# knights-lab/BURST

Hardware: AMD Instinct MI355X
Metric: aligned reads/sec (node), 100-bp synthetic reads @0.98 id vs RefSeq stand-in .edx/.acx (DB15), -m BEST; 1 GPU (higher is better)
Workload: dtype u32 bit-vectors (u8 edit distances)

## Files before the change

burst_amd/csrc/bhip_align.hip:

```cpp
#include "bhip_handle.h"
#include "bhip_pf_select.h"

__global__ void k_hit_count(const BhipHit *__restrict__ hits, uint32_t n, const uint32_t *__restrict__ n_dev, uint32_t *__restrict__ cnt, uint32_t *__restrict__ rank) {
	if (n_dev) n = *n_dev < n ? *n_dev : n;
	for (uint32_t i = blockIdx.x * blockDim.x + threadIdx.x; i < n; i += gridDim.x * blockDim.x) rank[i] = atomicAdd(&cnt[hits[i].q], 1u);
}
__global__ void k_hit_scatter(const BhipHit *__restrict__ in, uint32_t n, const uint32_t *__restrict__ n_dev, const uint32_t *__restrict__ off, const uint32_t *__restrict__ rank,
                              BhipHit *__restrict__ out, const uint32_t *__restrict__ qmap) {
	if (n_dev) n = *n_dev < n ? *n_dev : n;
	for (uint32_t i = blockIdx.x * blockDim.x + threadIdx.x; i < n; i += gridDim.x * blockDim.x) {
		BhipHit h = in[i];
		const uint32_t dst = off[h.q] + rank[i];
		if (qmap) h.q = qmap[h.q];
		out[dst] = h;
	}
}
__global__ void k_junk_adjust_raw(BhipRawHit *__restrict__ raw, const uint32_t *__restrict__ n_raw_dev, uint32_t raw_cap, const uint8_t *__restrict__ nx) {
	uint32_t n = *n_raw_dev;
	if (n > raw_cap) n = raw_cap;
	for (uint32_t i = blockIdx.x * blockDim.x + threadIdx.x; i < n; i += gridDim.x * blockDim.x) { const uint32_t x = nx[raw[i].q]; raw[i].ed += x; raw[i].m += x; }
}
__global__ void k_junk_adjust_best(uint32_t *__restrict__ best, const uint8_t *__restrict__ nx_six, uint32_t s0, uint32_t s1) {
	for (uint32_t s = s0 + blockIdx.x * blockDim.x + threadIdx.x; s < s1; s += gridDim.x * blockDim.x)
		if (nx_six[s] && best[s] != 0xFFFFFFFFu) best[s] += nx_six[s];
// ... 152 lines not shown
	memset(&fa, 0, sizeof fa);
	if (hipFuncGetAttributes(&fa, fn) != hipSuccess) return 4;
	return bhip_resident_blocks(threads, {fa.numRegs, fa.sharedSizeBytes}, dyn_lds);
}
template <auto FN> static BhipKernelRes kernel_res() {
	static const BhipKernelRes res = [] { hipFuncAttributes fa; memset(&fa, 0, sizeof fa);
		return hipFuncGetAttributes(&fa, (const void *)FN) == hipSuccess ? BhipKernelRes{fa.numRegs, fa.sharedSizeBytes} : BhipKernelRes{0, 0}; }();
	return res;
}

static void launch_window(Handle *h, Lane *L, hipStream_t wst, int cls, int NWP, uint32_t grid_cap, const BhipWin *wins, const uint32_t *n_wins, Counters *dc) {
	const uint32_t *six = six_or_null(h);
	const uint4 *ref = ref_args(h).chunks();
	const int NWc = kClasses[cls];
	const int min_class = h->opt_no_band ? 0 : NWc >= 8 ? 3 : NWc >= 6 ? 2 : NWc >= 4 ? 1 : 0;
	for_each_int(BwList{}, [&](auto bw) {
		constexpr int BW = decltype(bw)::value;
		if (min_class < BW - 1) return;
		uint32_t per_cu = blocks_per_cu((const void *)k_myers_window_band<BW>, 64u, 0);
		if (h->opt_band_blocks > 0) per_cu = (uint32_t)h->opt_band_blocks;
		const uint32_t grid = (uint32_t)h->n_cu * per_cu * (uint32_t)h->opt_oversub;
		hipLaunchKernelGGL(k_myers_window_band<BW>, dim3(grid), dim3(64), 0, wst, wins, n_wins, (uint32_t)L->win_cap, NWP, NWc, L->peq.as<uint32_t>(), six,
			ref, L->raw.as<BhipRawHit>(), &dc->n_raw, (uint32_t)L->raw_cap, h->best.as<uint32_t>(), &dc->wcol_sum, dc->win_class_seen);
	});
	dispatch_int(NwList{}, NWc, [&](auto nw) {
		constexpr int N = decltype(nw)::value;
		const uint32_t thr = N <= 8 ? 64u : 256u;
		const uint32_t grid = std::min<uint32_t>(grid_cap * (256u / thr), (uint32_t)h->n_cu * blocks_per_cu((const void *)k_myers_window<N>, thr, 0));
		hipLaunchKernelGGL(k_myers_window<N>, dim3(grid), dim3(thr), 0, wst, wins, n_wins, (uint32_t)L->win_cap, NWP, min_class, L->peq.as<uint32_t>(), six,
			ref, L->raw.as<BhipRawHit>(), &dc->n_raw, (uint32_t)L->raw_cap, h->best.as<uint32_t>(), &dc->wcol_sum, dc->win_class_seen);
	});
}


static int upload_queries(Handle *h, const uint8_t *q_codes, const uint64_t *q_off, const uint16_t *q_emac,
                          const uint32_t *q_six, const uint8_t *q_rc, uint32_t n_q) {
	const uint64_t nb = q_off[n_q];
	int rc;
	h->cur->st_has_junk = false;
	h->cur->st_maxlen = 0; h->cur->st_maxE = 0;
	for (uint32_t i = 0; i < n_q; ++i) {
		h->cur->st_maxlen = std::max<uint32_t>(h->cur->st_maxlen, (uint32_t)(q_off[i + 1] - q_off[i]));
		h->cur->st_maxE = std::max<uint32_t>(h->cur->st_maxE, q_emac[i]);
	}
	if ((rc = h->cur->qcodes.reserve(nb + 16))) return rc;
// ... 622 lines not shown
	for (uint32_t l = 0; l < b.nl; ++l) {
		Lane *L = h->lanes[l];
		const bool cq_min_only = !b.all_hits && h->opt_pf_cw == 2 && L->pf_algo_used == 3;
		if (L->n_entries && L->pf_algo == 0 && !cq_min_only && L->hc.ent_read > 100000 && (double)L->hc.surv_sum > (b.all_hits ? 0.20 : 0.50) * (double)L->hc.ent_read) L->pf_algo = 1;
	}
}
static void print_chain_counters(const Handle *h, const BatchCall &b) {
	for (uint32_t l = 0; l < b.nl; ++l) {
		const Lane *L = h->lanes[l];
		if (!L->n_entries) continue;
		fprintf(stderr, "[bhip] lane %u: %llu list records, %llu survived the counting filter, next prefilter algorithm %d\n", l, (unsigned long long)L->hc.ent_read, (unsigned long long)L->hc.surv_sum, L->pf_algo);
		for (int cls = 0; cls < kNumClasses; ++cls) if (L->npf[cls] + L->nex[cls])
			fprintf(stderr, "[bhip] lane %u class NW=%d: prefiltered %u exhaustive %u maxE %u maxwords %u | tasks %u + deferred %u (kept %u) clump pairs %u windows %u + %u | fallback queries(last class) %u raw %u\n",
				l, kClasses[cls], L->npf[cls], L->nex[cls], L->maxE[cls], L->maxwords[cls], L->hc.n_tasks_cls[cls], L->hc.n_tasks2_cls[cls], L->hc.n_tasks2k_cls[cls], L->hc.n_cand_cls[cls], L->hc.n_wins_cls[cls], L->hc.n_wins2_cls[cls], L->hc.n_fb, L->hc.n_raw);
		if (L->hc.n_fb) fprintf(stderr, "[bhip] lane %u: %u queries overflowed the first prefilter pass, %u the second (dense fallback)\n", l, L->hc.n_fb, L->hc.n_fb2);
		const uint32_t *rs = L->hc.n_rs;
		fprintf(stderr, "[bhip] lane %u: re-scorer bands 4:%u 6:%u 8:%u 12:%u 16:%u 24:%u 32:%u 40:%u 48:%u lds:%u scratch:%u\n",
			l, rs[0], rs[1], rs[2], rs[3], rs[4], rs[5], rs[6], rs[7], rs[8], rs[9], L->hc.n_wide);
		if (h->opt_rescore_reg) {
			static const char *const qf_name[BHIP_QF_COUNT] = {"dword", "lds", "chunk"};
			const BhipQueryFetch *f = L->qfetch;
			fprintf(stderr, "[bhip] lane %u: re-scorer query fetch 4-8:%s/%u 12:%s/%u 16-24:%s/%u 32-48:%s/%u\n", l, qf_name[f[0].form], f[0].lds_bytes,
				qf_name[f[3].form], f[3].lds_bytes, qf_name[f[1].form], f[1].lds_bytes, qf_name[f[2].form], f[2].lds_bytes);
		}
	}
}
static int grow_lane_capacities(Handle *h, const BatchCall &b) {
	bool redo = false;
	for (uint32_t l = 0; l < b.nl; ++l) {
		Lane *L = h->lanes[l];
// ... 337 lines not shown
```

burst_amd/csrc/bhip_handle.h:

```cpp
#ifndef BHIP_HANDLE_H
#define BHIP_HANDLE_H
#include <hip/hip_runtime.h>
#include <hipcub/hipcub.hpp>
#include <string>
#include <stdint.h>
#include <stdio.h>
#include <stdarg.h>
#include <stdlib.h>
#include <string.h>
#include <algorithm>
#include <vector>
#include <mutex>
#include <atomic>
#include <chrono>
#include <thread>
#include "burst_hip.h"
#include "bhip_internal.h"
#include "bhip_fetch_plan.h"

__global__ void k_acx_offsets(const uint32_t *, uint64_t, int, uint32_t *, unsigned long long *);
__global__ void k_acx_lines(const uint32_t *, uint64_t, int, unsigned long long *, uint4 *);
__global__ void k_acx_decode(const uint8_t *, const unsigned long long *, const uint32_t *, BhipAcxView, uint64_t, int, uint32_t, uint32_t *, uint32_t *);
__global__ void k_transpose_refs(const uint8_t *, const uint64_t *, const uint32_t *, const uint64_t *, uint32_t, uint4 *);
__global__ void k_build_peq(const uint8_t *, const uint64_t *, const uint32_t *, uint32_t, int, int, BhipMatchMask, uint32_t *, const uint32_t *, uint32_t, uint32_t);
// ... 3 lines not shown
__global__ void k_prefilter_hash(const uint8_t *, const uint64_t *, const uint16_t *, const uint32_t *, uint32_t, BhipAcxView, int,
	const uint32_t *, uint32_t, uint2 *, uint32_t *, uint32_t *, uint32_t, unsigned long long *, const uint32_t *, uint32_t *, uint32_t *);
template <typename CNT> __global__ void k_prefilter_wave(const uint8_t *, const uint64_t *, const uint16_t *, const uint32_t *, uint32_t,
	BhipAcxView, int, uint32_t, const uint32_t *, uint32_t, uint2 *, uint32_t *, uint32_t *, uint32_t, unsigned long long *, const uint32_t *,
	const uint32_t *, const uint32_t *);
template <int NW> __global__ void k_myers(const uint2 *, const uint32_t *, uint64_t, uint32_t, uint32_t, const uint32_t *, const uint32_t *,
	const uint64_t *, const uint16_t *, const uint32_t *, const uint4 *, const uint64_t *, const uint32_t *, uint32_t,
	BhipRawHit *, uint32_t *, uint32_t, uint32_t *, uint8_t *, unsigned long long *, unsigned long long *);
__global__ void k_myers_long(const uint2 *, const uint32_t *, uint64_t, uint32_t, uint32_t, const uint32_t *, const uint32_t *,
	const uint64_t *, const uint16_t *, const uint32_t *, const uint4 *, const uint64_t *, const uint32_t *, uint32_t,
	BhipRawHit *, uint32_t *, uint32_t, uint32_t *, uint8_t *, unsigned long long *, unsigned long long *, uint32_t);
template <int NWP> __global__ void k_myers_prefix(const uint2 *, const uint32_t *, uint64_t, uint32_t, uint32_t, const uint32_t *, const uint32_t *,
	const uint64_t *, const uint16_t *, const uint4 *, const uint64_t *, const uint32_t *, uint32_t, BhipWin *, uint32_t *, uint32_t,
	unsigned long long *, unsigned long long *, uint32_t *, const uint32_t *);
template <int NW> __global__ void k_myers_window(const BhipWin *, const uint32_t *, uint32_t, int, int, const uint32_t *, const uint32_t *,
	const uint4 *, BhipRawHit *, uint32_t *, uint32_t, uint32_t *, unsigned long long *, const uint32_t *);
template <int BW> __global__ void k_myers_window_band(const BhipWin *, const uint32_t *, uint32_t, int, int, const uint32_t *, const uint32_t *,
	const uint4 *, BhipRawHit *, uint32_t *, uint32_t, uint32_t *, unsigned long long *, const uint32_t *);
__global__ void k_extract_kmers(const uint4 *, const uint64_t *, const uint32_t *, const uint64_t *, uint32_t, uint32_t, int, unsigned long long *, uint16_t *, uint32_t *);
__global__ void k_attach_masks(BhipAcxView, uint64_t, const unsigned long long *, const uint16_t *, uint32_t, const uint32_t *, uint32_t *, uint32_t, uint32_t);
template <int HTB> __global__ void k_prefilter_mask(const uint2 *, const uint2 *, uint32_t, uint32_t, const uint32_t *, const uint32_t *, uint32_t, const uint32_t *, uint32_t,
	uint2 *, uint32_t *, uint32_t, unsigned long long *, uint32_t *, uint32_t *, unsigned long long *, unsigned long long *, unsigned long long *,
	uint2 *, uint32_t *, uint32_t);
template <int MODE, int BIG> __global__ void k_prefilter_cq(const uint2 *, const uint2 *, uint32_t, uint32_t, const uint32_t *, const uint32_t *, uint32_t, const uint32_t *, uint32_t,
	uint2 *, uint32_t *, uint32_t, unsigned long long *, uint32_t *, uint32_t *, unsigned long long *, unsigned long long *, unsigned long long *, unsigned long long *,
	uint2 *, uint32_t *, int, const uint32_t *, const uint32_t *, int);
template <int MODE, int BIG> __global__ void k_prefilter_cw(const uint2 *, const uint2 *, uint32_t, uint32_t, const uint32_t *, const uint32_t *, uint32_t, const uint32_t *, uint32_t,
	uint2 *, uint32_t *, uint32_t, unsigned long long *, uint32_t *, uint32_t *, unsigned long long *, unsigned long long *, unsigned long long *, unsigned long long *,
	uint2 *, uint32_t *, int, const uint32_t *, const uint32_t *, int);
__global__ void k_task_filter(const uint2 *, const uint32_t *, uint32_t, const uint32_t *, const uint32_t *, const uint32_t *, uint2 *, uint32_t *);
__global__ void k_seed_ranges(const uint8_t *, const uint64_t *, const uint32_t *, uint32_t, BhipAcxView, int, const uint32_t *, uint32_t, uint2 *, uint2 *, const uint32_t *, uint32_t, const uint16_t *, uint4 *, const uint32_t *, uint32_t, uint32_t, BhipAlt);
template <int NWP> __global__ void k_myers_prefix_task(const uint2 *, const uint32_t *, uint32_t, const uint32_t *, const uint32_t *, const uint64_t *,
	const uint16_t *, const uint4 *, const uint64_t *, const uint32_t *, BhipWin *, uint32_t *, uint32_t, unsigned long long *, uint32_t *, const uint4 *, const uint32_t *);
// ... 151 lines not shown

struct Counters {
	uint32_t n_cand, n_raw, n_out, n_wide, err, pad0;
	uint32_t n_cand_cls[8];
	uint32_t n_wins_cls[8];
	uint32_t n_fb, n_fb2;
	uint32_t n_tasks_cls[8];
	uint32_t n_tasks2_cls[8];
	uint32_t n_tasks2k_cls[8];
	uint32_t n_wins2_cls[8];
	uint32_t n_rs[12];
	unsigned long long wcol_sum, tcol_sum, unit_sum;
	unsigned long long col_sum, qlen_sum, ent_read, scratch_used;
	unsigned long long surv_sum;
	uint32_t win_class_seen[4];
};

struct StageSlot {
	DBuf qcodes, qcodes4, qlen16, qoff, qemac, qsix, qrc, qflags, qmap, off_raw, plan, qpack, key, key_sorted, idx, idx_sorted, sort_tmp, info;
	DBuf qcodes_s, qoff_s, qemac_s, qpack_s, nx, nx_six;
	BhipStageInfo *info_pinned = nullptr;
	hipEvent_t ev_begin = nullptr, ev_done = nullptr, ev_copied = nullptr;
	int state = 0;
	uint64_t seq = 0;
	bool resolved = false;
	bool st_valid = false, st_has_six = false, st_has_rc = false, st_has_junk = false, has_flags = false, has_qmap = false;
	uint32_t st_nq = 0, st_nshared = 0, st_maxlen = 0, st_maxE = 0, st_lanes = 1;
	float st_ms_h2d = 0, st_ms_copy = 0, st_ms_route = 0;
	std::vector<BhipQuerySpan> spans;
	const uint32_t *six_explicit = nullptr;
// ... 94 lines not shown
	const uint16_t *s_emac() const { return cur->st_has_junk ? cur->qemac_s.as<uint16_t>() : cur->qemac.as<uint16_t>(); }
	const uint32_t *s_pack() const { return cur->st_has_junk ? cur->qpack_s.as<uint32_t>() : cur->qpack.as<uint32_t>(); }
	DBuf sort_keys, sort_keys2, sort_idx, sort_tmp, out_sorted, out_sorted2, sort_scratch;
	uint64_t out_cap = 1 << 20;
	std::vector<uint32_t> h_clump_len;
	BhipStats stats;
	std::vector<Lane *> lanes;
	int opt_two_stage = 1;
	int opt_prefilter_stride = 0;
	int opt_lanes = 1;
	int opt_sweep_blocks = 8;
	uint32_t peq_rows = 16;
	int opt_oversub = 2;
	int opt_band_blocks = 0;
	int opt_no_band = 0;
	int opt_async_d2h = 0, out_idx = 0;
	hipStream_t copy_stream = nullptr;
	hipEvent_t ev_sorted = nullptr, ev_copied[2] = {nullptr, nullptr};
	bool copy_pending[2] = {false, false};
	void *reg_ptr[2] = {nullptr, nullptr}; size_t reg_bytes[2] = {0, 0};
	int last_out = 0;
	uint64_t last_n_out = 0;
	int opt_prune = 1;
	int opt_lane_min = 32768;
	int opt_rescore_reg = 1;
	int opt_fetch_once = 1;
	int opt_pf_waves = 0;
	int opt_pf_algo = -1;
	int opt_pf_table = 0;
	int opt_pf_cw = 2;
// ... 39 lines not shown
```

burst_amd/csrc/bhip_init.hip:

```cpp
#include "bhip_handle.h"

static thread_local char g_err[512] = "";

__global__ void k_ref_symbol_scan(const uint32_t *__restrict__ w, uint64_t n_words, uint32_t *__restrict__ flag) {
	uint32_t any = 0;
	for (uint64_t i = blockIdx.x * (uint64_t)blockDim.x + threadIdx.x; i < n_words; i += (uint64_t)gridDim.x * blockDim.x) {
		const uint32_t d = w[i];
		any |= (d | ((d << 1) & ((d << 2) | (d << 3)))) & 0x88888888u;
	}
	if (any) *flag = 1u;
}
int bhip_fail_msg(int code, const char *fmt, ...) {
	va_list ap; va_start(ap, fmt); vsnprintf(g_err, sizeof g_err, fmt, ap); va_end(ap);
	return code;
}

extern "C" const char *bhip_last_error(void) { return g_err; }
extern "C" int bhip_abi_version(void) { return BHIP_ABI_VERSION; }
std::atomic<int> &bhip_vmm_peer_access_flag() { return bhip_vmm_peer_access(); }

static void lane_destroy(Lane *L) {
	if (!L) return;
	DBuf *all[] = {&L->peq, &L->peqp, &L->cand, &L->candcnt, &L->wins, &L->raw, &L->wide, &L->scratch, &L->fb_list, &L->gcnt, &L->counters, &L->tasks, &L->tasks2, &L->tasks2k, &L->wins2, &L->rs_lists};
	for (DBuf *b : all) b->release();
// ... 185 lines not shown
		h->opt_prefilter_stride = (int)value; return BHIP_OK;
	}
	if (!strcmp(name, "two_stage")) { h->opt_two_stage = value != 0; return BHIP_OK; }
	if (!strcmp(name, "host_routing")) { h->opt_host_routing = value != 0; return BHIP_OK; }
	if (!strcmp(name, "discard_staged")) { for (StageSlot &S : h->slots) if (S.state == 1) S.state = 0; h->res_valid = false; return BHIP_OK; }
	if (!strcmp(name, "lane_masks")) { h->opt_lane_masks = value != 0; return BHIP_OK; }
	if (!strcmp(name, "sweep_blocks")) { if (value < 1 || value > 8) return fail(BHIP_E_ARG, "sweep_blocks must be 1 .. 8"); h->opt_sweep_blocks = (int)value; return BHIP_OK; }
	if (!strcmp(name, "lane_min_entries")) { if (value < 1) return fail(BHIP_E_ARG, "lane_min_entries must be >= 1"); h->opt_lane_min = (int)value; return BHIP_OK; }
	if (!strcmp(name, "async_d2h")) { h->opt_async_d2h = value != 0; return BHIP_OK; }
	if (!strcmp(name, "seed_ahead")) { h->opt_seed_ahead = value != 0; return BHIP_OK; }
	if (!strcmp(name, "peq_ahead_blocks")) { if (value < 1 || value > 16) return fail(BHIP_E_ARG, "peq_ahead_blocks must be 1 .. 16"); h->opt_peq_ahead_blocks = (int)value; return BHIP_OK; }
	if (!strcmp(name, "seed_ahead_blocks")) { if (value < 0 || value > 64) return fail(BHIP_E_ARG, "seed_ahead_blocks must be 0 .. 64"); h->opt_seed_ahead_blocks = (int)value; return BHIP_OK; }
	if (!strcmp(name, "band_blocks")) { if (value < 0 || value > 1024) return fail(BHIP_E_ARG, "band_blocks must be 0 .. 1024"); h->opt_band_blocks = (int)value; return BHIP_OK; }
	if (!strcmp(name, "oversub")) { if (value < 1 || value > 16) return fail(BHIP_E_ARG, "oversub must be 1 .. 16"); h->opt_oversub = (int)value; return BHIP_OK; }
	if (!strcmp(name, "band")) { h->opt_no_band = value == 0; return BHIP_OK; }
	if (!strcmp(name, "prune")) { h->opt_prune = value != 0; return BHIP_OK; }
	if (!strcmp(name, "rescore_reg")) { h->opt_rescore_reg = value != 0; return BHIP_OK; }
	if (!strcmp(name, "fetch_once")) { h->opt_fetch_once = value != 0; return BHIP_OK; }
	if (!strcmp(name, "seed_min_need")) { if (value < -1 || value > 255) return fail(BHIP_E_ARG, "seed_min_need must be -1 (by rule) or 0 .. 255"); h->opt_seed_min_need = (int)value; return BHIP_OK; }
	if (!strcmp(name, "seed_drop_len")) { if (value < 0 || value > (1 << 24)) return fail(BHIP_E_ARG, "seed_drop_len must be 0 .. 2^24"); h->opt_seed_drop_len = (int)value; return BHIP_OK; }
	if (!strcmp(name, "prefilter_waves")) { if (value < 0 || value > 16) return fail(BHIP_E_ARG, "prefilter_waves must be 0 .. 16"); h->opt_pf_waves = (int)value; return BHIP_OK; }
	if (!strcmp(name, "prefilter_algo")) { if (value < -1 || value > 1) return fail(BHIP_E_ARG, "prefilter_algo must be -1, 0 or 1"); h->opt_pf_algo = (int)value; return BHIP_OK; }
	if (!strcmp(name, "prefilter_table")) { if (value != 0 && (value < 9 || value > 11)) return fail(BHIP_E_ARG, "prefilter_table must be 0, 9, 10 or 11"); h->opt_pf_table = (int)value; return BHIP_OK; }
	if (!strcmp(name, "prefilter_cw")) { if (value < 0 || value > 2) return fail(BHIP_E_ARG, "prefilter_cw must be 0, 1 or 2"); h->opt_pf_cw = (int)value; return BHIP_OK; }
	if (!strcmp(name, "prefilter_bytes")) { h->opt_pf_bytes = value != 0; return BHIP_OK; }
	if (!strcmp(name, "prefilter_rb")) { if (value != 0 && (value < 2 || value > 4)) return fail(BHIP_E_ARG, "prefilter_rb must be 0, 2, 3 or 4"); h->opt_pf_rb = (int)value; return BHIP_OK; }
	if (!strcmp(name, "cov_event_cap")) { if (value < 0) return fail(BHIP_E_ARG, "cov_event_cap must be >= 0 bytes (0 = a fifth of the free memory)"); h->opt_cov_event_cap = value; return BHIP_OK; }
	if (!strcmp(name, "em_weak_hash")) { h->opt_em_weak_hash = value != 0; return BHIP_OK; }
	if (!strcmp(name, "em_thread_max")) { if (value < 0 || value > 64) return fail(BHIP_E_ARG, "em_thread_max must be 0 (built in) .. 64"); h->opt_em_thread_max = (int)value; return BHIP_OK; }
	if (!strcmp(name, "em_wave_max")) { if (value < 0 || value > (1 << 24)) return fail(BHIP_E_ARG, "em_wave_max must be 0 (built in) .. 2^24"); h->opt_em_wave_max = (int)value; return BHIP_OK; }
// ... 19 lines not shown
```

burst_amd/csrc/bhip_internal.h:

```cpp
#ifndef BHIP_INTERNAL_H
#define BHIP_INTERNAL_H
#include <stdint.h>

struct BhipMatchMask { uint16_t m[16]; };

struct BhipRawHit {
	uint32_t q;
	uint32_t refIx;
	uint32_t ed;
	uint32_t e_first;
	uint32_t e_last;
	uint32_t m;
	uint32_t L;
	uint32_t six;
	uint64_t rbase;
};

#define BHIP_WIN_GMASK 0x3FFFFFFFu
struct BhipWin {
	uint32_t li;
	uint32_t refIx;
	uint32_t g_first, g_last;
	uint32_t q;
	uint32_t mE;
	uint32_t nchunks;
	uint32_t L;
	uint64_t rbase;
	uint32_t six;
	uint32_t pad2;
};
__host__ __device__ inline uint32_t bhip_win_class(uint32_t g_first, uint32_t g_last, uint32_t E) {
	const uint64_t diags = 8ull * (g_last - g_first) + 8u + 2u * E;
	return diags <= 26 ? 0u : diags <= 58 ? 1u : diags <= 90 ? 2u : 3u;
}

#define BHIP_PLAN_STRIDE(p) ((p) & 255u)
#define BHIP_PLAN_NEED(p)   (((p) >> 8) & 0xFFFFu)
#define BHIP_PLAN_X(p)      (((p) >> 24) & 15u)
#define BHIP_PLAN_USED(p)   ((p) >> 28)
#define BHIP_EXPAND_SLOTS 8u
struct BhipAlt { uint8_t n[16]; uint8_t base[16]; };

template <class Sym>
__host__ __device__ inline uint32_t bhip_word_class(Sym sym, uint32_t p, uint32_t K, const BhipAlt &A, uint32_t &amb_k, uint32_t &extra) {
	uint32_t namb = 0, bad = 0;
	amb_k = 0; extra = 0;
	for (uint32_t k = 0; k < K; ++k) {
		const uint32_t n = A.n[sym(p + k) & 15u];
		if (n == 0u) bad = 1u;
// ... 82 lines not shown
```

burst_amd/csrc/bhip_kernels.hip:

```cpp
#include <hip/hip_runtime.h>
#include <stdint.h>
#include <type_traits>
#include "burst_hip.h"
#include "bhip_internal.h"
#include "bhip_fetch_plan.h"

__global__ void k_transpose_refs(const uint8_t *__restrict__ src, const uint64_t *__restrict__ src_off,
                                 const uint32_t *__restrict__ clump_len, const uint64_t *__restrict__ dst_off,
                                 uint32_t n_clumps, uint4 *__restrict__ dst_lane) {
	const uint32_t z = threadIdx.x & 15, g = threadIdx.x >> 4, gpb = blockDim.x >> 4;
	for (uint32_t c = blockIdx.x; c < n_clumps; c += gridDim.x) {
		const uint32_t L = clump_len[c], nrows = (L + 1) >> 1, nchunks = (L + 31) >> 5;
		const uint8_t *s = src + src_off[c] * 16;
		for (uint32_t t = g; t < nchunks; t += gpb) {
			uint32_t w[4] = {0, 0, 0, 0};
			#pragma unroll
			for (int i = 0; i < 16; ++i) {
				uint32_t row = 16 * t + i;
				uint32_t b = row < nrows ? s[(uint64_t)row * 16 + z] : 0u;
				w[i >> 2] |= b << (8 * (i & 3));
			}
			dst_lane[dst_off[c] * 16 + (uint64_t)z * nchunks + t] = make_uint4(w[0], w[1], w[2], w[3]);
		}
	}
// ... 457 lines not shown
		for (int t = 0; t < 8; ++t) if (keep[t]) out[s_base + rank[t]] = tk[t];
		__syncthreads();
	}
}

#define BHIP_INST_PREFIX_TASK(NWP) \
	template __global__ void k_myers_prefix_task<NWP>(const uint2 *, const uint32_t *, uint32_t, const uint32_t *, const uint32_t *, const uint64_t *, \
		const uint16_t *, const uint4 *, const uint64_t *, const uint32_t *, BhipWin *, uint32_t *, uint32_t, unsigned long long *, uint32_t *, const uint4 *, const uint32_t *);
BHIP_INST_PREFIX_TASK(1) BHIP_INST_PREFIX_TASK(2) BHIP_INST_PREFIX_TASK(3) BHIP_INST_PREFIX_TASK(4) BHIP_INST_PREFIX_TASK(6)

template <int NW>
__global__ __launch_bounds__(256) void k_myers_window(
		const BhipWin *__restrict__ wins, const uint32_t *__restrict__ n_wins_dev, uint32_t win_cap, int NWP, int min_class,
		const uint32_t *__restrict__ peq, const uint32_t *__restrict__ qsix, const uint4 *__restrict__ ref,
		BhipRawHit *__restrict__ raw, uint32_t *__restrict__ n_raw, uint32_t raw_cap, uint32_t *__restrict__ best,
		unsigned long long *__restrict__ wcol_sum, const uint32_t *__restrict__ cls_seen) {
	if (min_class > 0) {
		uint32_t any = 0;
		for (int c = min_class; c < 4; ++c) any |= cls_seen[c];
		if (!any) return;
	}
	constexpr bool LDS_TAB = NW <= 8;
	__shared__ uint32_t s_tab[LDS_TAB ? 4 * NW : 1][LDS_TAB ? 64 : 1];
	uint32_t n = *n_wins_dev;
	if (n > win_cap) n = win_cap;
	unsigned long long my_cols = 0;
	for (uint32_t i = blockIdx.x * blockDim.x + threadIdx.x; i < n; i += gridDim.x * blockDim.x) {
		const BhipWin w = wins[i];
		if ((int)(w.g_first >> 30) < min_class) continue;
		const uint32_t li = w.li, q = w.q;
		const uint32_t m = w.mE & 0xFFFFu, E = w.mE >> 16;
		const uint32_t P = m < 32u * (uint32_t)NWP ? m : 32u * (uint32_t)NWP;
		const uint32_t nchunks = w.nchunks, gA8 = w.g_first & BHIP_WIN_GMASK;
		const int col_lo = (int)(gA8 * 8 + 2) - (int)(P + E), col_hi = (int)((w.g_last + 1) * 8 + (m - P) + E);
		const uint32_t c_lo = col_lo > 1 ? (uint32_t)(col_lo - 1) : 0u;
		uint32_t c_hi = (uint32_t)(col_hi - 1);
		if (c_hi >= nchunks * 32) c_hi = nchunks * 32 - 1;
		const uint32_t tA = c_lo >> 5, tB = c_hi >> 5, gA = (c_lo & 31u) >> 3, gE = (c_hi & 31u) >> 3;
		uint32_t Pv[NW], Mv[NW];
		#pragma unroll
		for (int k = 0; k < NW; ++k) {
			const int lo = 32 * NW - (int)m - 32 * k;
			Pv[k] = lo <= 0 ? 0xFFFFFFFFu : (lo >= 32 ? 0u : (0xFFFFFFFFu << lo));
			Mv[k] = 0;
// ... 33 lines not shown
				}
			}
		}
		my_cols += ((tB * 4 + gE) - (tA * 4 + gA) + 1) * 8;
		if ((uint32_t)bestS <= E) {
			const uint32_t pos = atomicAdd(n_raw, 1u);
			if (pos < raw_cap) {
				BhipRawHit h; h.q = q; h.refIx = w.refIx; h.ed = (uint32_t)bestS; h.e_first = first; h.e_last = last;
				h.m = m; h.L = w.L; h.six = w.six; h.rbase = w.rbase;
				raw[pos] = h;
			}
			if (best) atomicMin(&best[w.six], (uint32_t)bestS);
		}
	}
	if (wcol_sum && my_cols) atomicAdd(wcol_sum, my_cols);
}

template <int BW>
__global__ __launch_bounds__(64) void k_myers_window_band(
		const BhipWin *__restrict__ wins, const uint32_t *__restrict__ n_wins_dev, uint32_t win_cap, int NWP, int NW,
		const uint32_t *__restrict__ peq, const uint32_t *__restrict__ qsix, const uint4 *__restrict__ ref,
		BhipRawHit *__restrict__ raw, uint32_t *__restrict__ n_raw, uint32_t raw_cap, uint32_t *__restrict__ best,
		unsigned long long *__restrict__ wcol_sum, const uint32_t *__restrict__ cls_seen) {
	if (BW > 2 && !cls_seen[BW - 2]) return;
	__shared__ uint32_t s_tab[4 * BW][64];
	const uint32_t tid = threadIdx.x;
	uint32_t n = *n_wins_dev;
	if (n > win_cap) n = win_cap;
	unsigned long long my_cols = 0;
#ifndef WB_PREFETCH
#define WB_PREFETCH 0
#endif
#if WB_PREFETCH
	BhipWin w_next;
	if (blockIdx.x * 64u + tid < n) w_next = wins[blockIdx.x * 64u + tid];
#endif
	for (uint32_t i = blockIdx.x * 64u + tid; i < n; i += gridDim.x * 64u) {
#if WB_PREFETCH
		const BhipWin w = w_next;
		if (i + gridDim.x * 64u < n) w_next = wins[i + gridDim.x * 64u];
#else
		const BhipWin w = wins[i];
#endif
		if (w.g_first >> 30 != (uint32_t)(BW - 2)) continue;
		const uint32_t m = w.mE & 0xFFFFu, E = w.mE >> 16, g_first = w.g_first & BHIP_WIN_GMASK;
		const uint32_t P = m < 32u * (uint32_t)NWP ? m : 32u * (uint32_t)NWP;
		const uint32_t nchunks = w.nchunks;
		const int col_lo = (int)(g_first * 8 + 2) - (int)(P + E), col_hi = (int)((w.g_last + 1) * 8 + (m - P) + E);
		const uint32_t c_lo = col_lo > 1 ? (uint32_t)(col_lo - 1) : 0u;
		uint32_t c_hi = (uint32_t)(col_hi - 1);
		if (c_hi >= nchunks * 32) c_hi = nchunks * 32 - 1;
		const uint32_t jA = c_lo >> 3, jB = c_hi >> 3, tB = jB >> 2;
		const int dmax = (int)(w.g_last * 8 + 8) - (int)P + (int)E;
		const int shift = 32 * NW - (int)m;
		int ylo = (int)(jA * 8 + 1) - dmax; if (ylo < 0) ylo = 0;
		int wb = (shift - 1 + ylo) >> 5;
		wb = wb < 0 ? 0 : (wb > NW - BW ? NW - BW : wb);
		auto init_word = [&](int k) -> uint32_t { const int lo = shift - 32 * k; return lo <= 0 ? 0xFFFFFFFFu : (lo >= 32 ? 0u : (0xFFFFFFFFu << lo)); };
		uint32_t Pb[BW], Mb[BW];
		#pragma unroll
// ... 98 lines not shown
				if (tcur < tB) { const uint4 v = rp[tcur + 1]; n0 = v.x; n1 = v.y; n2 = v.z; n3 = v.w; }
			} else { c0 = c1; c1 = c2; c2 = c3; }
		}
		my_cols += (jB - jA + 1) * 8;
		if ((uint32_t)bestS <= E) {
			const uint32_t pos = atomicAdd(n_raw, 1u);
			if (pos < raw_cap) {
				BhipRawHit h; h.q = w.q; h.refIx = w.refIx; h.ed = (uint32_t)bestS; h.e_first = first; h.e_last = last;
				h.m = m; h.L = w.L; h.six = w.six; h.rbase = w.rbase;
				raw[pos] = h;
			}
			if (best) atomicMin(&best[w.six], (uint32_t)bestS);
		}
	}
	if (wcol_sum && my_cols) atomicAdd(wcol_sum, my_cols);
}
#define BHIP_INST_BAND(BW) \
	template __global__ void k_myers_window_band<BW>(const BhipWin *, const uint32_t *, uint32_t, int, int, const uint32_t *, const uint32_t *, \
		const uint4 *, BhipRawHit *, uint32_t *, uint32_t, uint32_t *, unsigned long long *, const uint32_t *);
BHIP_INST_BAND(2) BHIP_INST_BAND(3) BHIP_INST_BAND(4)

#define BHIP_INST_PREFIX(NWP) \
	template __global__ void k_myers_prefix<NWP>(const uint2 *, const uint32_t *, uint64_t, uint32_t, uint32_t, const uint32_t *, const uint32_t *, \
		const uint64_t *, const uint16_t *, const uint4 *, const uint64_t *, const uint32_t *, uint32_t, BhipWin *, uint32_t *, uint32_t, \
		unsigned long long *, unsigned long long *, uint32_t *, const uint32_t *);
BHIP_INST_PREFIX(1) BHIP_INST_PREFIX(2) BHIP_INST_PREFIX(3) BHIP_INST_PREFIX(4) BHIP_INST_PREFIX(6)
#define BHIP_INST_WINDOW(NW) \
	template __global__ void k_myers_window<NW>(const BhipWin *, const uint32_t *, uint32_t, int, int, const uint32_t *, const uint32_t *, \
		const uint4 *, BhipRawHit *, uint32_t *, uint32_t, uint32_t *, unsigned long long *, const uint32_t *);
BHIP_INST_WINDOW(2) BHIP_INST_WINDOW(4) BHIP_INST_WINDOW(6) BHIP_INST_WINDOW(8) BHIP_INST_WINDOW(10) BHIP_INST_WINDOW(16) BHIP_INST_WINDOW(32)

#define BHIP_INST_MYERS(NW) \
	template __global__ void k_myers<NW>(const uint2 *, const uint32_t *, uint64_t, uint32_t, uint32_t, const uint32_t *, const uint32_t *, \
		const uint64_t *, const uint16_t *, const uint32_t *, const uint4 *, const uint64_t *, const uint32_t *, uint32_t, \
		BhipRawHit *, uint32_t *, uint32_t, uint32_t *, uint8_t *, unsigned long long *, unsigned long long *);
BHIP_INST_MYERS(2) BHIP_INST_MYERS(4) BHIP_INST_MYERS(6) BHIP_INST_MYERS(8) BHIP_INST_MYERS(10)
BHIP_INST_MYERS(16) BHIP_INST_MYERS(32)

__device__ __forceinline__ uint32_t sat8u(uint32_t v) { return v > 255u ? 255u : v; }

__device__ __forceinline__ uint4 ref_chunk_lane(const uint32_t *__restrict__ refw_lane, uint64_t clump_base, uint32_t z, int t4, uint32_t nchunks) {
	if (t4 < 0 || (uint32_t)t4 >= nchunks) return make_uint4(0, 0, 0, 0);
	return ((const uint4 *)refw_lane)[clump_base * 16 + (uint64_t)z * nchunks + (uint32_t)t4];
}
// ... 641 lines not shown
```

Before: 621.9 million.

## Add single-word band kernel for narrow Myers verification windows

Adds a k_myers_window_band1 kernel that verifies windows whose diagonal span fits in one 32-bit word (at most 25 diagonals), tracking a single sliding P/M word instead of the 2-word band. The existing band-2 and full-window kernels skip windows that band1 handles. They return early when band1 reports nothing left over. Per-sweep counters are added for diagnostics. This cuts per-column bit-vector work for the common narrow windows of high-identity reads, at the cost of an extra launch, some atomics and added complexity in the sliding-offset bookkeeping.

```diff
diff --git a/burst_amd/csrc/bhip_align.hip b/burst_amd/csrc/bhip_align.hip
--- a/burst_amd/csrc/bhip_align.hip
+++ b/burst_amd/csrc/bhip_align.hip
@@ -190,6 +190,14 @@
 	const uint4 *ref = ref_args(h).chunks();
 	const int NWc = kClasses[cls];
 	const int min_class = h->opt_no_band ? 0 : NWc >= 8 ? 3 : NWc >= 6 ? 2 : NWc >= 4 ? 1 : 0;
+	const int band1 = !h->opt_no_band && h->opt_band1 && NWc <= 32;
+	if (band1) {
+		uint32_t per_cu = blocks_per_cu((const void *)k_myers_window_band1, 64u, 0);
+		if (h->opt_band_blocks > 0) per_cu = (uint32_t)h->opt_band_blocks;
+		const uint32_t grid = (uint32_t)h->n_cu * per_cu * (uint32_t)h->opt_oversub;
+		hipLaunchKernelGGL(k_myers_window_band1, dim3(grid), dim3(64), 0, wst, wins, n_wins, (uint32_t)L->win_cap, NWP, NWc, L->peq.as<uint32_t>(), six,
+			ref, L->raw.as<BhipRawHit>(), &dc->n_raw, (uint32_t)L->raw_cap, h->best.as<uint32_t>(), &dc->wcol_sum, dc->n_sweep);
+	}
 	for_each_int(BwList{}, [&](auto bw) {
 		constexpr int BW = decltype(bw)::value;
 		if (min_class < BW - 1) return;
@@ -197,14 +205,14 @@
 		if (h->opt_band_blocks > 0) per_cu = (uint32_t)h->opt_band_blocks;
 		const uint32_t grid = (uint32_t)h->n_cu * per_cu * (uint32_t)h->opt_oversub;
 		hipLaunchKernelGGL(k_myers_window_band<BW>, dim3(grid), dim3(64), 0, wst, wins, n_wins, (uint32_t)L->win_cap, NWP, NWc, L->peq.as<uint32_t>(), six,
-			ref, L->raw.as<BhipRawHit>(), &dc->n_raw, (uint32_t)L->raw_cap, h->best.as<uint32_t>(), &dc->wcol_sum, dc->win_class_seen);
+			ref, L->raw.as<BhipRawHit>(), &dc->n_raw, (uint32_t)L->raw_cap, h->best.as<uint32_t>(), &dc->wcol_sum, dc->win_class_seen, dc->n_sweep, BW == 2 ? band1 : 0);
 	});
 	dispatch_int(NwList{}, NWc, [&](auto nw) {
 		constexpr int N = decltype(nw)::value;
 		const uint32_t thr = N <= 8 ? 64u : 256u;
 		const uint32_t grid = std::min<uint32_t>(grid_cap * (256u / thr), (uint32_t)h->n_cu * blocks_per_cu((const void *)k_myers_window<N>, thr, 0));
 		hipLaunchKernelGGL(k_myers_window<N>, dim3(grid), dim3(thr), 0, wst, wins, n_wins, (uint32_t)L->win_cap, NWP, min_class, L->peq.as<uint32_t>(), six,
-			ref, L->raw.as<BhipRawHit>(), &dc->n_raw, (uint32_t)L->raw_cap, h->best.as<uint32_t>(), &dc->wcol_sum, dc->win_class_seen);
+			ref, L->raw.as<BhipRawHit>(), &dc->n_raw, (uint32_t)L->raw_cap, h->best.as<uint32_t>(), &dc->wcol_sum, dc->win_class_seen, dc->n_sweep, min_class == 0 ? band1 : 0);
 	});
 }
 
@@ -857,6 +865,8 @@
 			fprintf(stderr, "[bhip] lane %u class NW=%d: prefiltered %u exhaustive %u maxE %u maxwords %u | tasks %u + deferred %u (kept %u) clump pairs %u windows %u + %u | fallback queries(last class) %u raw %u\n",
 				l, kClasses[cls], L->npf[cls], L->nex[cls], L->maxE[cls], L->maxwords[cls], L->hc.n_tasks_cls[cls], L->hc.n_tasks2_cls[cls], L->hc.n_tasks2k_cls[cls], L->hc.n_cand_cls[cls], L->hc.n_wins_cls[cls], L->hc.n_wins2_cls[cls], L->hc.n_fb, L->hc.n_raw);
 		if (L->hc.n_fb) fprintf(stderr, "[bhip] lane %u: %u queries overflowed the first prefilter pass, %u the second (dense fallback)\n", l, L->hc.n_fb, L->hc.n_fb2);
+		const uint32_t *sw = L->hc.n_sweep;
+		fprintf(stderr, "[bhip] lane %u: window sweeps band1:%u band2:%u band3:%u band4:%u full:%u\n", l, sw[BHIP_SWEEP_BAND1], sw[BHIP_SWEEP_BAND2], sw[BHIP_SWEEP_BAND3], sw[BHIP_SWEEP_BAND4], sw[BHIP_SWEEP_FULL]);
 		const uint32_t *rs = L->hc.n_rs;
 		fprintf(stderr, "[bhip] lane %u: re-scorer bands 4:%u 6:%u 8:%u 12:%u 16:%u 24:%u 32:%u 40:%u 48:%u lds:%u scratch:%u\n",
 			l, rs[0], rs[1], rs[2], rs[3], rs[4], rs[5], rs[6], rs[7], rs[8], rs[9], L->hc.n_wide);
diff --git a/burst_amd/csrc/bhip_band1_plan.h b/burst_amd/csrc/bhip_band1_plan.h
--- /dev/null
+++ b/burst_amd/csrc/bhip_band1_plan.h
@@ -0,0 +1,50 @@
+#ifndef BHIP_BAND1_PLAN_H
+#define BHIP_BAND1_PLAN_H
+#include <stdint.h>
+
+#ifdef __HIPCC__
+#define BHIP_B1_FN __host__ __device__ inline
+#else
+#define BHIP_B1_FN static inline
+#endif
+
+#define BHIP_BAND1_MAX_DIAGS 25u
+BHIP_B1_FN uint64_t bhip_band1_diags(uint32_t g_first, uint32_t g_last, uint32_t E) { return 8ull * (g_last - g_first) + 8u + 2ull * E; }
+BHIP_B1_FN bool bhip_band1_takes(uint32_t g_first, uint32_t g_last, uint32_t E) { return g_last >= g_first && bhip_band1_diags(g_first, g_last, E) <= BHIP_BAND1_MAX_DIAGS; }
+
+BHIP_B1_FN void bhip_window_dwords(uint32_t g_first, uint32_t g_last, uint32_t m, uint32_t P, uint32_t E, uint32_t nchunks, uint32_t &jA, uint32_t &jB) {
+	const int col_lo = (int)(g_first * 8 + 2) - (int)(P + E), col_hi = (int)((g_last + 1) * 8 + (m - P) + E);
+	const uint32_t c_lo = col_lo > 1 ? (uint32_t)(col_lo - 1) : 0u;
+	uint32_t c_hi = (uint32_t)(col_hi - 1);
+	if (c_hi >= nchunks * 32) c_hi = nchunks * 32 - 1;
+	jA = c_lo >> 3; jB = c_hi >> 3;
+}
+
+struct BhipBand1 {
+	int shift;
+	int dmax;
+	int omax;
+};
+BHIP_B1_FN BhipBand1 bhip_band1_make(int NW, uint32_t m, uint32_t P, uint32_t E, uint32_t g_last) {
+	BhipBand1 b;
+	b.shift = 32 * NW - (int)m;
+	b.dmax = (int)(g_last * 8 + 8) - (int)P + (int)E;
+	b.omax = 32 * (NW - 1);
+	return b;
+}
+BHIP_B1_FN int bhip_band1_offset(const BhipBand1 &b, uint32_t col0) {
+	const int v = b.shift + (int)col0 - b.dmax - 1;
+	return v < 0 ? 0 : (v > b.omax ? b.omax : v);
+}
+BHIP_B1_FN uint32_t bhip_band1_init_p(const BhipBand1 &b, int o) {
+	const int lo = b.shift - o;
+	return lo <= 0 ? 0xFFFFFFFFu : (lo >= 32 ? 0u : (0xFFFFFFFFu << lo));
+}
+BHIP_B1_FN int bhip_band1_init_score(const BhipBand1 &b, int o) { const int s = o + 32 - b.shift; return s < 0 ? 0 : s; }
+BHIP_B1_FN uint32_t bhip_band1_carry(const BhipBand1 &b, int o) { return o > b.shift ? 1u : 0u; }
+BHIP_B1_FN uint32_t bhip_band1_fresh(const BhipBand1 &b, int o, uint32_t s) {
+	const uint32_t all = (1u << s) - 1u;
+	const int lo = b.shift - (o + 32);
+	return lo <= 0 ? all : (lo >= (int)s ? 0u : (all & (0xFFFFFFFFu << lo)));
+}
+#endif
diff --git a/burst_amd/csrc/bhip_handle.h b/burst_amd/csrc/bhip_handle.h
--- a/burst_amd/csrc/bhip_handle.h
+++ b/burst_amd/csrc/bhip_handle.h
@@ -41,9 +41,11 @@
 	const uint64_t *, const uint16_t *, const uint4 *, const uint64_t *, const uint32_t *, uint32_t, BhipWin *, uint32_t *, uint32_t,
 	unsigned long long *, unsigned long long *, uint32_t *, const uint32_t *);
 template <int NW> __global__ void k_myers_window(const BhipWin *, const uint32_t *, uint32_t, int, int, const uint32_t *, const uint32_t *,
-	const uint4 *, BhipRawHit *, uint32_t *, uint32_t, uint32_t *, unsigned long long *, const uint32_t *);
+	const uint4 *, BhipRawHit *, uint32_t *, uint32_t, uint32_t *, unsigned long long *, const uint32_t *, uint32_t *, int);
 template <int BW> __global__ void k_myers_window_band(const BhipWin *, const uint32_t *, uint32_t, int, int, const uint32_t *, const uint32_t *,
-	const uint4 *, BhipRawHit *, uint32_t *, uint32_t, uint32_t *, unsigned long long *, const uint32_t *);
+	const uint4 *, BhipRawHit *, uint32_t *, uint32_t, uint32_t *, unsigned long long *, const uint32_t *, uint32_t *, int);
+__global__ void k_myers_window_band1(const BhipWin *, const uint32_t *, uint32_t, int, int, const uint32_t *, const uint32_t *,
+	const uint4 *, BhipRawHit *, uint32_t *, uint32_t, uint32_t *, unsigned long long *, uint32_t *);
 __global__ void k_extract_kmers(const uint4 *, const uint64_t *, const uint32_t *, const uint64_t *, uint32_t, uint32_t, int, unsigned long long *, uint16_t *, uint32_t *);
 __global__ void k_attach_masks(BhipAcxView, uint64_t, const unsigned long long *, const uint16_t *, uint32_t, const uint32_t *, uint32_t *, uint32_t, uint32_t);
 template <int HTB> __global__ void k_prefilter_mask(const uint2 *, const uint2 *, uint32_t, uint32_t, const uint32_t *, const uint32_t *, uint32_t, const uint32_t *, uint32_t,
@@ -225,6 +227,8 @@
 	unsigned long long col_sum, qlen_sum, ent_read, scratch_used;
 	unsigned long long surv_sum;
 	uint32_t win_class_seen[4];
+	uint32_t n_sweep[BHIP_SWEEP_COUNT];
+	uint32_t pad1[2];
 };
 
 struct StageSlot {
@@ -349,6 +353,7 @@
 	int opt_oversub = 2;
 	int opt_band_blocks = 0;
 	int opt_no_band = 0;
+	int opt_band1 = 1;
 	int opt_async_d2h = 0, out_idx = 0;
 	hipStream_t copy_stream = nullptr;
 	hipEvent_t ev_sorted = nullptr, ev_copied[2] = {nullptr, nullptr};
diff --git a/burst_amd/csrc/bhip_init.hip b/burst_amd/csrc/bhip_init.hip
--- a/burst_amd/csrc/bhip_init.hip
+++ b/burst_amd/csrc/bhip_init.hip
@@ -223,6 +223,7 @@
 	if (!strcmp(name, "band_blocks")) { if (value < 0 || value > 1024) return fail(BHIP_E_ARG, "band_blocks must be 0 .. 1024"); h->opt_band_blocks = (int)value; return BHIP_OK; }
 	if (!strcmp(name, "oversub")) { if (value < 1 || value > 16) return fail(BHIP_E_ARG, "oversub must be 1 .. 16"); h->opt_oversub = (int)value; return BHIP_OK; }
 	if (!strcmp(name, "band")) { h->opt_no_band = value == 0; return BHIP_OK; }
+	if (!strcmp(name, "band1")) { h->opt_band1 = value != 0; return BHIP_OK; }
 	if (!strcmp(name, "prune")) { h->opt_prune = value != 0; return BHIP_OK; }
 	if (!strcmp(name, "rescore_reg")) { h->opt_rescore_reg = value != 0; return BHIP_OK; }
 	if (!strcmp(name, "fetch_once")) { h->opt_fetch_once = value != 0; return BHIP_OK; }
diff --git a/burst_amd/csrc/bhip_internal.h b/burst_amd/csrc/bhip_internal.h
--- a/burst_amd/csrc/bhip_internal.h
+++ b/burst_amd/csrc/bhip_internal.h
@@ -33,6 +33,8 @@
 	const uint64_t diags = 8ull * (g_last - g_first) + 8u + 2u * E;
 	return diags <= 26 ? 0u : diags <= 58 ? 1u : diags <= 90 ? 2u : 3u;
 }
+
+enum { BHIP_SWEEP_BAND1 = 0, BHIP_SWEEP_BAND2 = 1, BHIP_SWEEP_BAND3 = 2, BHIP_SWEEP_BAND4 = 3, BHIP_SWEEP_FULL = 4, BHIP_SWEEP_LEFT = 5, BHIP_SWEEP_COUNT = 6 };
 
 #define BHIP_PLAN_STRIDE(p) ((p) & 255u)
 #define BHIP_PLAN_NEED(p)   (((p) >> 8) & 0xFFFFu)
diff --git a/burst_amd/csrc/bhip_kernels.hip b/burst_amd/csrc/bhip_kernels.hip
--- a/burst_amd/csrc/bhip_kernels.hip
+++ b/burst_amd/csrc/bhip_kernels.hip
@@ -4,6 +4,7 @@
 #include "burst_hip.h"
 #include "bhip_internal.h"
 #include "bhip_fetch_plan.h"
+#include "bhip_band1_plan.h"
 
 __global__ void k_transpose_refs(const uint8_t *__restrict__ src, const uint64_t *__restrict__ src_off,
                                  const uint32_t *__restrict__ clump_len, const uint64_t *__restrict__ dst_off,
@@ -495,10 +496,10 @@
 		const BhipWin *__restrict__ wins, const uint32_t *__restrict__ n_wins_dev, uint32_t win_cap, int NWP, int min_class,
 		const uint32_t *__restrict__ peq, const uint32_t *__restrict__ qsix, const uint4 *__restrict__ ref,
 		BhipRawHit *__restrict__ raw, uint32_t *__restrict__ n_raw, uint32_t raw_cap, uint32_t *__restrict__ best,
-		unsigned long long *__restrict__ wcol_sum, const uint32_t *__restrict__ cls_seen) {
-	if (min_class > 0) {
-		uint32_t any = 0;
-		for (int c = min_class; c < 4; ++c) any |= cls_seen[c];
+		unsigned long long *__restrict__ wcol_sum, const uint32_t *__restrict__ cls_seen, uint32_t *__restrict__ sweep_ctr, int skip_band1) {
+	if (min_class > 0 || skip_band1) {
+		uint32_t any = min_class > 0 ? 0u : sweep_ctr[BHIP_SWEEP_LEFT];
+		for (int c = min_class > 1 ? min_class : 1; c < 4; ++c) any |= cls_seen[c];
 		if (!any) return;
 	}
 	constexpr bool LDS_TAB = NW <= 8;
@@ -506,9 +507,12 @@
 	uint32_t n = *n_wins_dev;
 	if (n > win_cap) n = win_cap;
 	unsigned long long my_cols = 0;
+	uint32_t my_wins = 0;
 	for (uint32_t i = blockIdx.x * blockDim.x + threadIdx.x; i < n; i += gridDim.x * blockDim.x) {
 		const BhipWin w = wins[i];
 		if ((int)(w.g_first >> 30) < min_class) continue;
+		if (skip_band1 && w.g_first >> 30 == 0u && bhip_band1_takes(w.g_first & BHIP_WIN_GMASK, w.g_last, w.mE >> 16)) continue;
+		++my_wins;
 		const uint32_t li = w.li, q = w.q;
 		const uint32_t m = w.mE & 0xFFFFu, E = w.mE >> 16;
 		const uint32_t P = m < 32u * (uint32_t)NWP ? m : 32u * (uint32_t)NWP;
@@ -572,6 +576,7 @@
 		}
 	}
 	if (wcol_sum && my_cols) atomicAdd(wcol_sum, my_cols);
+	if (my_wins) atomicAdd(&sweep_ctr[BHIP_SWEEP_FULL], my_wins);
 }
 
 template <int BW>
@@ -579,13 +584,15 @@
 		const BhipWin *__restrict__ wins, const uint32_t *__restrict__ n_wins_dev, uint32_t win_cap, int NWP, int NW,
 		const uint32_t *__restrict__ peq, const uint32_t *__restrict__ qsix, const uint4 *__restrict__ ref,
 		BhipRawHit *__restrict__ raw, uint32_t *__restrict__ n_raw, uint32_t raw_cap, uint32_t *__restrict__ best,
-		unsigned long long *__restrict__ wcol_sum, const uint32_t *__restrict__ cls_seen) {
+		unsigned long long *__restrict__ wcol_sum, const uint32_t *__restrict__ cls_seen, uint32_t *__restrict__ sweep_ctr, int skip_band1) {
 	if (BW > 2 && !cls_seen[BW - 2]) return;
+	if (BW == 2 && skip_band1 && !sweep_ctr[BHIP_SWEEP_LEFT]) return;
 	__shared__ uint32_t s_tab[4 * BW][64];
 	const uint32_t tid = threadIdx.x;
 	uint32_t n = *n_wins_dev;
 	if (n > win_cap) n = win_cap;
 	unsigned long long my_cols = 0;
+	uint32_t my_wins = 0;
 #ifndef WB_PREFETCH
 #define WB_PREFETCH 0
 #endif
@@ -602,6 +609,8 @@
 #endif
 		if (w.g_first >> 30 != (uint32_t)(BW - 2)) continue;
 		const uint32_t m = w.mE & 0xFFFFu, E = w.mE >> 16, g_first = w.g_first & BHIP_WIN_GMASK;
+		if (BW == 2 && skip_band1 && bhip_band1_takes(g_first, w.g_last, E)) continue;
+		++my_wins;
 		const uint32_t P = m < 32u * (uint32_t)NWP ? m : 32u * (uint32_t)NWP;
 		const uint32_t nchunks = w.nchunks;
 		const int col_lo = (int)(g_first * 8 + 2) - (int)(P + E), col_hi = (int)((w.g_last + 1) * 8 + (m - P) + E);
@@ -730,11 +739,133 @@
 		}
 	}
 	if (wcol_sum && my_cols) atomicAdd(wcol_sum, my_cols);
+	if (my_wins) atomicAdd(&sweep_ctr[BW - 1], my_wins);
 }
 #define BHIP_INST_BAND(BW) \
 	template __global__ void k_myers_window_band<BW>(const BhipWin *, const uint32_t *, uint32_t, int, int, const uint32_t *, const uint32_t *, \
-		const uint4 *, BhipRawHit *, uint32_t *, uint32_t, uint32_t *, unsigned long long *, const uint32_t *);
+		const uint4 *, BhipRawHit *, uint32_t *, uint32_t, uint32_t *, unsigned long long *, const uint32_t *, uint32_t *, int);
 BHIP_INST_BAND(2) BHIP_INST_BAND(3) BHIP_INST_BAND(4)
+
+__global__ __launch_bounds__(64, 7) void k_myers_window_band1(
+		const BhipWin *__restrict__ wins, const uint32_t *__restrict__ n_wins_dev, uint32_t win_cap, int NWP, int NW,
+		const uint32_t *__restrict__ peq, const uint32_t *__restrict__ qsix, const uint4 *__restrict__ ref,
+		BhipRawHit *__restrict__ raw, uint32_t *__restrict__ n_raw, uint32_t raw_cap, uint32_t *__restrict__ best,
+		unsigned long long *__restrict__ wcol_sum, uint32_t *__restrict__ sweep_ctr) {
+	__shared__ uint32_t s_tab[4][64];
+	const uint32_t tid = threadIdx.x;
+	uint32_t n = *n_wins_dev;
+	if (n > win_cap) n = win_cap;
+	unsigned long long my_cols = 0;
+	uint32_t my_wins = 0, my_left = 0;
+	for (uint32_t i = blockIdx.x * 64u + tid; i < n; i += gridDim.x * 64u) {
+		const BhipWin w = wins[i];
+		if (w.g_first >> 30 != 0u) continue;
+		const uint32_t m = w.mE & 0xFFFFu, E = w.mE >> 16, g_first = w.g_first & BHIP_WIN_GMASK;
+		if (!bhip_band1_takes(g_first, w.g_last, E)) { ++my_left; continue; }
+		++my_wins;
+		const uint32_t P = m < 32u * (uint32_t)NWP ? m : 32u * (uint32_t)NWP;
+		uint32_t jA, jB;
+		bhip_window_dwords(g_first, w.g_last, m, P, E, w.nchunks, jA, jB);
+		const uint32_t tB = jB >> 2;
+		const BhipBand1 B = bhip_band1_make(NW, m, P, E, w.g_last);
+		int o = bhip_band1_offset(B, jA * 8 + 1);
+		uint32_t Pb = bhip_band1_init_p(B, o), Mb = 0;
+		int sc = bhip_band1_init_score(B, o);
+		uint32_t hb = bhip_band1_carry(B, o);
+		bool top = o == B.omax;
+		int bestS = 0x7FFFFFFF;
+		uint32_t first = 0, last = 0;
+		const uint4 *rp = ref + w.rbase;
+		const uint32_t *tab = peq + (uint64_t)w.li * 16 * (uint32_t)NW;
+		int wq = o >> 5;
+		uint32_t lo[4], hi[4], nx[4];
+		#pragma unroll
+		for (int r = 0; r < 4; ++r) {
+			lo[r] = tab[(r + 1) * NW + wq];
+			hi[r] = tab[(r + 1) * NW + (wq + 1 < NW ? wq + 1 : NW - 1)];
+			nx[r] = tab[(r + 1) * NW + (wq + 2 < NW ? wq + 2 : NW - 1)];
+			s_tab[r][tid] = __builtin_amdgcn_alignbit(hi[r], lo[r], (uint32_t)o & 31u);
+		}
+		auto step = [&](auto track, uint32_t Eq, uint32_t col) {
+			const uint32_t sum = (Eq & Pb) + Pb;
+			const uint32_t Xh = (sum ^ Pb) | Eq;
+			uint32_t Ph = Mb | ~(Xh | Pb), Mh = Pb & Xh;
+			sc += (int)(Ph >> 31) + ((int)Mh >> 31);
+			Ph = Ph << 1 | hb; Mh <<= 1;
+			const uint32_t Xv = Eq | Mb;
+			Pb = Mh | ~(Xv | Ph);
+			Mb = Ph & Xv;
+			if constexpr (decltype(track)::value) {
+				const bool lt = sc < bestS, le = sc <= bestS;
+				bestS = lt ? sc : bestS;
+				first = lt ? col : first;
+				last = le ? col : last;
+			}
+		};
+		auto sweep8 = [&](auto track, uint32_t d, uint32_t col0) {
+			const uint32_t dm = d - 0x11111111u;
+			if ((dm & 0xCCCCCCCCu) == 0) {
+				uint32_t Eq[8];
+				#pragma unroll
+				for (int k8 = 0; k8 < 8; ++k8) Eq[k8] = s_tab[(dm >> (4 * k8)) & 3u][tid];
+				#pragma unroll
+				for (int k8 = 0; k8 < 8; ++k8) step(track, Eq[k8], col0 + (uint32_t)k8);
+			} else {
+				const int wh = wq + 1 < NW ? wq + 1 : NW - 1;
+				#pragma unroll
+				for (int k8 = 0; k8 < 8; ++k8) {
+					const uint32_t sym = (d >> (4 * k8)) & 15u;
+					step(track, __builtin_amdgcn_alignbit(tab[sym * NW + wh], tab[sym * NW + wq], (uint32_t)o & 31u), col0 + (uint32_t)k8);
+				}
+			}
+		};
+		uint32_t tcur = jA >> 2;
+		uint32_t c0, c1, c2, c3, n0, n1, n2, n3;
+		{ const uint4 v = rp[tcur]; c0 = v.x; c1 = v.y; c2 = v.z; c3 = v.w; }
+		{ const uint4 v = tcur < tB ? rp[tcur + 1] : make_uint4(0, 0, 0, 0); n0 = v.x; n1 = v.y; n2 = v.z; n3 = v.w; }
+		for (uint32_t r = 0; r < (jA & 3u); ++r) { c0 = c1; c1 = c2; c2 = c3; }
+		for (uint32_t j = jA; j <= jB; ++j) {
+			const uint32_t d = c0;
+			const uint32_t col0 = j * 8 + 1;
+			const int on = bhip_band1_offset(B, col0);
+			if (on != o) {
+				const uint32_t s = (uint32_t)(on - o);
+				const uint32_t fresh = bhip_band1_fresh(B, o, s);
+				Pb = Pb >> s | fresh << (32u - s);
+				Mb >>= s;
+				sc += __popc(fresh);
+				hb = bhip_band1_carry(B, on);
+				top = on == B.omax;
+				o = on;
+				if ((o >> 5) != wq) {
+					++wq;
+					#pragma unroll
+					for (int r = 0; r < 4; ++r) { lo[r] = hi[r]; hi[r] = nx[r]; nx[r] = tab[(r + 1) * NW + (wq + 2 < NW ? wq + 2 : NW - 1)]; }
+				}
+				#pragma unroll
+				for (int r = 0; r < 4; ++r) s_tab[r][tid] = __builtin_amdgcn_alignbit(hi[r], lo[r], (uint32_t)o & 31u);
+			}
+			if (top) sweep8(std::true_type(), d, col0); else sweep8(std::false_type(), d, col0);
+			if ((j & 3u) == 3u) {
+				c0 = n0; c1 = n1; c2 = n2; c3 = n3; ++tcur;
+				if (tcur < tB) { const uint4 v = rp[tcur + 1]; n0 = v.x; n1 = v.y; n2 = v.z; n3 = v.w; }
+			} else { c0 = c1; c1 = c2; c2 = c3; }
+		}
+		my_cols += (jB - jA + 1) * 8;
+		if ((uint32_t)bestS <= E) {
+			const uint32_t pos = atomicAdd(n_raw, 1u);
+			if (pos < raw_cap) {
+				BhipRawHit h; h.q = w.q; h.refIx = w.refIx; h.ed = (uint32_t)bestS; h.e_first = first; h.e_last = last;
+				h.m = m; h.L = w.L; h.six = w.six; h.rbase = w.rbase;
+				raw[pos] = h;
+			}
+			if (best) atomicMin(&best[w.six], (uint32_t)bestS);
+		}
+	}
+	if (wcol_sum && my_cols) atomicAdd(wcol_sum, my_cols);
+	if (my_wins) atomicAdd(&sweep_ctr[BHIP_SWEEP_BAND1], my_wins);
+	if (my_left) atomicAdd(&sweep_ctr[BHIP_SWEEP_LEFT], my_left);
+}
 
 #define BHIP_INST_PREFIX(NWP) \
 	template __global__ void k_myers_prefix<NWP>(const uint2 *, const uint32_t *, uint64_t, uint32_t, uint32_t, const uint32_t *, const uint32_t *, \
@@ -743,7 +874,7 @@
 BHIP_INST_PREFIX(1) BHIP_INST_PREFIX(2) BHIP_INST_PREFIX(3) BHIP_INST_PREFIX(4) BHIP_INST_PREFIX(6)
 #define BHIP_INST_WINDOW(NW) \
 	template __global__ void k_myers_window<NW>(const BhipWin *, const uint32_t *, uint32_t, int, int, const uint32_t *, const uint32_t *, \
-		const uint4 *, BhipRawHit *, uint32_t *, uint32_t, uint32_t *, unsigned long long *, const uint32_t *);
+		const uint4 *, BhipRawHit *, uint32_t *, uint32_t, uint32_t *, unsigned long long *, const uint32_t *, uint32_t *, int);
 BHIP_INST_WINDOW(2) BHIP_INST_WINDOW(4) BHIP_INST_WINDOW(6) BHIP_INST_WINDOW(8) BHIP_INST_WINDOW(10) BHIP_INST_WINDOW(16) BHIP_INST_WINDOW(32)
 
 #define BHIP_INST_MYERS(NW) \
```

After: 609.2 million. 0.98x the previous value.
